# arkworks-rs/groth16

Measured on NVIDIA H100. Metric: groth16_proofs_per_sec_bls12_381_2^20, higher is better.
Workload: dtype u32 limbs (255-bit Fr / 381-bit Fq Montgomery integers)

## Files before the change

### groth16_b200/api.py

```python
from __future__ import annotations

import ctypes as C
from dataclasses import dataclass, field
from typing import List, Optional, Sequence, Tuple

import numpy as np

from . import _lib
from .codec import CurveCodec
from .params import CurveParams, get_curve


class SynthesisError(Exception):
    """ark_relations::r1cs::SynthesisError"""


class PolynomialDegreeTooLarge(SynthesisError):
    pass


class MalformedKey(SynthesisError):
    pass


# ... 278 lines not shown

    def prove_wait_raw(self, slot: int, out: np.ndarray):
        _check(self._lib.g16_prove_wait(self._ctx, slot, _ptr(out)))

    def prove_partial_submit_raw(self, slot: int, r_limbs: np.ndarray, z_ptr, flags: int):
        _check(self._lib.g16_prove_partial_submit(self._ctx, slot, _ptr(r_limbs), C.c_void_p(z_ptr), flags))

    def prove_partial_wait_raw(self, slot: int, out: np.ndarray):
        _check(self._lib.g16_prove_partial_wait(self._ctx, slot, _ptr(out)))

    def prove_partial_raw(self, r_limbs: np.ndarray, z_ptr, flags: int, out: np.ndarray):
        _check(self._lib.g16_prove_partial(self._ctx, _ptr(r_limbs), C.c_void_p(z_ptr), flags, _ptr(out)))

    def comm_unique_id(self) -> np.ndarray:
        out = np.zeros(256, dtype=np.uint8)
        _check(self._lib.g16_comm_unique_id(out.ctypes.data_as(C.c_void_p)))
        return out

    def comm_init(self, unique_id: np.ndarray, rank: int, world: int):
        uid = np.ascontiguousarray(unique_id, dtype=np.uint8)
        assert uid.size == 256
        _check(self._lib.g16_comm_init(self._ctx, uid.ctypes.data_as(C.c_void_p), rank, world))

    def prove_sharded_raw(self, r_limbs, s_limbs, z_ptr, flags: int, out: np.ndarray):
        _check(self._lib.g16_prove_sharded(self._ctx, _ptr(r_limbs), _ptr(s_limbs), C.c_void_p(z_ptr), flags, _ptr(out)))

    def prove_sharded_submit_raw(self, slot: int, r_limbs, s_limbs, z_ptr, flags: int):
        _check(self._lib.g16_prove_sharded_submit(self._ctx, slot, _ptr(r_limbs), _ptr(s_limbs), C.c_void_p(z_ptr), flags))

    def prove_sharded_wait_raw(self, slot: int, out: np.ndarray):
        _check(self._lib.g16_prove_sharded_wait(self._ctx, slot, _ptr(out)))

    def prove_assemble_prepare(self, r, s):
        self._asm_keep = (self._fr_arg(r), self._fr_arg(s))
        _check(self._lib.g16_prove_assemble_prepare(self._ctx, _ptr(self._asm_keep[0]), _ptr(self._asm_keep[1])))

    def prove_assemble(self, r, s, partials: np.ndarray) -> Proof:
        rr, ss = self._fr_arg(r), self._fr_arg(s)
        pl = self._lib.g16_partial_limbs(self._ctx)
        p = np.ascontiguousarray(partials, dtype=np.uint64).reshape(-1, pl)
        nq = self.nq
        out = np.zeros(8 * nq, dtype=np.uint64)
        _check(self._lib.g16_prove_assemble(self._ctx, _ptr(rr), _ptr(ss), _ptr(p), p.shape[0], _ptr(out)))
        return Proof(out[:2 * nq].copy(), out[2 * nq:6 * nq].copy(), out[6 * nq:].copy())

    def partial_limbs(self) -> int:
        return self._lib.g16_partial_limbs(self._ctx)

    def witness_map_from_matrices(self, matrices: Optional[ConstraintMatrices], num_inputs: int, num_constraints: int,
                                  full_assignment: np.ndarray) -> np.ndarray:
        if matrices is not None and matrices is not self._matrices:
            self.load_matrices(matrices)
        m = self._matrices
        z = np.ascontiguousarray(full_assignment, dtype=np.uint64).reshape(-1, 4)
        if z.shape[0] != m.num_instance_variables + m.num_witness_variables:
            raise ValueError("full_assignment has the wrong length")
        n = 1 << self._lib.g16_domain_log(self._ctx)
        h = np.zeros((n, 4), dtype=np.uint64)
        _check(self._lib.g16_witness_map(self._ctx, _ptr(z), 0, _ptr(h)))
        return h

    def timings(self) -> dict:
        t = _lib.Timings()
        _check(self._lib.g16_get_timings(self._ctx, C.byref(t)))
        names = ["h", "l", "a", "b_g1", "b_g2"]
        return dict(total_ms=t.total_ms, h2d_ms=t.h2d_ms, witness_map_ms=t.witness_map_ms,
                    msm_ms={n: t.msm_ms[i] for i, n in enumerate(names)},
                    msm_accum_ms={n: t.msm_accum_ms[i] for i, n in enumerate(names)},
                    msm_pairs={n: int(t.msm_pairs[i]) for i, n in enumerate(names)},
                    msm_entries={n: int(t.msm_entries[i]) for i, n in enumerate(names)},
                    msm_begin_ms={n: t.msm_begin_ms[i] for i, n in enumerate(names)},
                    msm_end_ms={n: t.msm_end_ms[i] for i, n in enumerate(names)},
                    host_finish_ms=t.host_finish_ms, launches=int(t.launches), h2d_bytes=int(t.h2d_bytes),
                    d2h_bytes=int(t.d2h_bytes))

    def set_option(self, key: str, value: int):
        _check(self._lib.g16_set_option(self._ctx, key.encode(), int(value)))

    def config(self) -> dict:
        c = _lib.Config()
        _check(self._lib.g16_get_config(self._ctx, C.byref(c)))
        d = {n: int(getattr(c, n)) for n, _ in _lib.Config._fields_ if n != "reserved"}
        R = d["ba_rounds_g1"]
        ba_mul = 6.0 + 3.0 / max(1, d["ba_m"])
        frac = 1.0 - 0.5 ** R
        d["imad_per_g1_entry_mul"] = frac * ba_mul + (1.0 - frac) * 10.0 if R > 0 else 10.0
        d["g1_accum_stage"] = (f"G1 bucket accumulation: {R} batched-affine rounds (ba_forward / ba_combine / ba_backward) + "
                               "msm_accum_l0<Fq> on the last list; one stage per G1 MSM" if R > 0 else
                               "msm_accum_l0<Fq> (G1 bucket accumulation, XYZZ mixed additions); one launch per G1 MSM")
        return d

    def _fr_arg(self, x) -> np.ndarray:
        if isinstance(x, (int, np.integer)):
            return np.ascontiguousarray(self.codec.fr.enc1(int(x)))
        return np.ascontiguousarray(x, dtype=np.uint64).reshape(4)
```

### groth16_b200/csrc/ec.cuh

```cuda
#pragma once
#include "fp.cuh"

#ifdef __CUDACC__
#define G16_HD_NOINLINE __host__ __device__ __noinline__
#else
#define G16_HD_NOINLINE
#endif

namespace g16 {

template <class P, int NR>
struct alignas(16) Fp2 {
  using B = Fp<P>;
  B c0, c1;
  G16_HD static Fp2 zero() { return {B::zero(), B::zero()}; }
  G16_HD static Fp2 one() { return {B::one(), B::zero()}; }
  G16_HD bool is_zero() const { return c0.is_zero() && c1.is_zero(); }
  G16_HD bool operator==(const Fp2& o) const { return c0 == o.c0 && c1 == o.c1; }
  G16_HD bool operator!=(const Fp2& o) const { return !(*this == o); }
  G16_HD static Fp2 add(const Fp2& a, const Fp2& b) { return {B::add(a.c0, b.c0), B::add(a.c1, b.c1)}; }
  G16_HD static Fp2 sub(const Fp2& a, const Fp2& b) { return {B::sub(a.c0, b.c0), B::sub(a.c1, b.c1)}; }
  G16_HD static Fp2 neg(const Fp2& a) { return {B::neg(a.c0), B::neg(a.c1)}; }
  G16_HD static Fp2 dbl(const Fp2& a) { return {B::dbl(a.c0), B::dbl(a.c1)}; }
  G16_HD static B mul_nr(const B& a) { return NR == 1 ? a : B::mul_small(a, NR); }
  G16_HD static Fp2 mul(const Fp2& a, const Fp2& b) {
    B v0 = B::mul(a.c0, b.c0);
    B v1 = B::mul(a.c1, b.c1);
    B s = B::mul(B::add(a.c0, a.c1), B::add(b.c0, b.c1));
    Fp2 r;
    r.c0 = B::sub(v0, mul_nr(v1));
    r.c1 = B::sub(B::sub(s, v0), v1);
    return r;
  }
  G16_HD static Fp2 sqr(const Fp2& a) {
    B t = B::mul(a.c0, a.c1);
    B s = B::mul(B::add(a.c0, a.c1), B::sub(a.c0, mul_nr(a.c1)));
    Fp2 r;
    r.c0 = (NR == 1) ? s : B::add(s, B::mul_small(t, NR - 1));
    r.c1 = B::dbl(t);
    return r;
  }
  G16_HD static Fp2 mul_small(const Fp2& a, int k) { return {B::mul_small(a.c0, k), B::mul_small(a.c1, k)}; }
  G16_HD static Fp2 inv(const Fp2& a) {
    B n = B::add(B::sqr(a.c0), mul_nr(B::sqr(a.c1)));
    B ni = B::inv(n);
    return {B::mul(a.c0, ni), B::neg(B::mul(a.c1, ni))};
  }
};

template <class F>
struct alignas(16) Affine {
  F x, y;
  G16_HD bool is_inf() const { return x.is_zero() && y.is_zero(); }
  G16_HD static Affine inf() { return {F::zero(), F::zero()}; }
};

template <class F>
struct alignas(16) XYZZ {
  F X, Y, ZZ, ZZZ;
  G16_HD bool is_inf() const { return ZZ.is_zero(); }
  G16_HD static XYZZ inf() { return {F::zero(), F::zero(), F::zero(), F::zero()}; }
  G16_HD static XYZZ from_affine(const Affine<F>& p) {
    if (p.is_inf()) return inf();
    return {p.x, p.y, F::one(), F::one()};
  }

  G16_HD_NOINLINE static XYZZ dbl_affine(const Affine<F>& p) {
    if (p.is_inf() || p.y.is_zero()) return inf();
    F U = F::dbl(p.y);
    F V = F::sqr(U);
    F W = F::mul(U, V);
    F S = F::mul(p.x, V);
    F XX = F::sqr(p.x);
    F M = F::add(F::dbl(XX), XX);
    XYZZ r;
    r.X = F::sub(F::sqr(M), F::dbl(S));
    r.Y = F::sub(F::mul(M, F::sub(S, r.X)), F::mul(W, p.y));
    r.ZZ = V;
    r.ZZZ = W;
    return r;
  }
  G16_HD_NOINLINE void dbl_inplace() {
    if (is_inf()) return;
    if (Y.is_zero()) { *this = inf(); return; }
    F U = F::dbl(Y);
    F V = F::sqr(U);
    F W = F::mul(U, V);
    F S = F::mul(X, V);
    F XX = F::sqr(X);
    F M = F::add(F::dbl(XX), XX);
    F X3 = F::sub(F::sqr(M), F::dbl(S));
    F Y3 = F::sub(F::mul(M, F::sub(S, X3)), F::mul(W, Y));
    X = X3;
    Y = Y3;
    ZZ = F::mul(V, ZZ);
    ZZZ = F::mul(W, ZZZ);
  }
  G16_HD_NOINLINE void madd(const Affine<F>& p_in, bool neg = false) { madd_inline(p_in, neg); }
  G16_HD void madd_inline(const Affine<F>& p_in, bool neg = false) {
    if (p_in.is_inf()) return;
    Affine<F> p = p_in;
    if (neg) p.y = F::neg(p.y);
    if (is_inf()) {
      X = p.x; Y = p.y; ZZ = F::one(); ZZZ = F::one();
      return;
    }
    F Pd = F::sub(F::mul(p.x, ZZ), X);
    F R = F::sub(F::mul(p.y, ZZZ), Y);
    if (Pd.is_zero()) {
      if (R.is_zero()) *this = dbl_affine(p);
      else *this = inf();
      return;
    }
    F PP = F::sqr(Pd);
    F PPP = F::mul(Pd, PP);
    F Q = F::mul(X, PP);
    F X3 = F::sub(F::sub(F::sqr(R), PPP), F::dbl(Q));
    Y = F::sub(F::mul(R, F::sub(Q, X3)), F::mul(Y, PPP));
    X = X3;
    ZZ = F::mul(ZZ, PP);
    ZZZ = F::mul(ZZZ, PPP);
  }
  template <class LX, class LY>
  G16_HD void madd_lazy(LX load_x, LY load_y, bool neg) {
    const F px = load_x();
    if (is_inf()) {
      F py = load_y();
      if (px.is_zero() && py.is_zero()) return;
      if (neg) py = F::neg(py);
      X = px; Y = py; ZZ = F::one(); ZZZ = F::one();
      return;
    }
    const F Pd = F::sub(F::mul(px, ZZ), X);
    F py = load_y();
    if (px.is_zero() && py.is_zero()) return;
    if (neg) py = F::neg(py);
    const F R = F::sub(F::mul(py, ZZZ), Y);
    if (Pd.is_zero()) {
      if (R.is_zero()) *this = dbl_affine(Affine<F>{px, py});
      else *this = inf();
      return;
    }
    const F PP = F::sqr(Pd);
    const F PPP = F::mul(Pd, PP);
    const F Q = F::mul(X, PP);
    const F X3 = F::sub(F::sub(F::sqr(R), PPP), F::dbl(Q));
    Y = F::sub(F::mul(R, F::sub(Q, X3)), F::mul(Y, PPP));
    X = X3;
    ZZ = F::mul(ZZ, PP);
    ZZZ = F::mul(ZZZ, PPP);
  }
  G16_HD_NOINLINE void add(const XYZZ& q) {
    if (q.is_inf()) return;
    if (is_inf()) { *this = q; return; }
    F U1 = F::mul(X, q.ZZ);
    F U2 = F::mul(q.X, ZZ);
    F S1 = F::mul(Y, q.ZZZ);
    F S2 = F::mul(q.Y, ZZZ);
    F Pd = F::sub(U2, U1);
    F R = F::sub(S2, S1);
    if (Pd.is_zero()) {
      if (R.is_zero()) dbl_inplace();
      else *this = inf();
      return;
    }
    F PP = F::sqr(Pd);
    F PPP = F::mul(Pd, PP);
    F Q = F::mul(U1, PP);
    F X3 = F::sub(F::sub(F::sqr(R), PPP), F::dbl(Q));
    Y = F::sub(F::mul(R, F::sub(Q, X3)), F::mul(S1, PPP));
    X = X3;
    ZZ = F::mul(F::mul(ZZ, q.ZZ), PP);
    ZZZ = F::mul(F::mul(ZZZ, q.ZZZ), PPP);
  }
  G16_HD void negate() { Y = F::neg(Y); }

  G16_HD_NOINLINE XYZZ mul_u32(const uint32_t* k, int nl) const {
    XYZZ r = inf();
    bool started = false;
    for (int i = nl * 32 - 1; i >= 0; i--) {
      if (started) r.dbl_inplace();
      if ((k[i >> 5] >> (i & 31)) & 1) {
        r.add(*this);
        started = true;
      }
    }
    return r;
  }
  G16_HD_NOINLINE Affine<F> to_affine() const {
    if (is_inf()) return Affine<F>::inf();
    F zi = F::inv(ZZZ);
    F z = F::mul(zi, ZZ);
    F zi2 = F::sqr(z);
    return {F::mul(X, zi2), F::mul(Y, zi)};
  }
};

}
```

### groth16_b200/csrc/fp.cuh

```cuda
#pragma once
#include <cstdint>
#include <cstring>
#include "g16_constants.h"

namespace g16 {

#if defined(__CUDA_ARCH__)
#define G16_PTX_PATH 1
namespace ptx {
__device__ __forceinline__ void add_cc(uint32_t& r, uint32_t a, uint32_t b) { asm volatile("add.cc.u32 %0, %1, %2;" : "=r"(r) : "r"(a), "r"(b)); }
__device__ __forceinline__ void addc_cc(uint32_t& r, uint32_t a, uint32_t b) { asm volatile("addc.cc.u32 %0, %1, %2;" : "=r"(r) : "r"(a), "r"(b)); }
__device__ __forceinline__ void addc(uint32_t& r, uint32_t a, uint32_t b) { asm volatile("addc.u32 %0, %1, %2;" : "=r"(r) : "r"(a), "r"(b)); }
__device__ __forceinline__ void sub_cc(uint32_t& r, uint32_t a, uint32_t b) { asm volatile("sub.cc.u32 %0, %1, %2;" : "=r"(r) : "r"(a), "r"(b)); }
__device__ __forceinline__ void subc_cc(uint32_t& r, uint32_t a, uint32_t b) { asm volatile("subc.cc.u32 %0, %1, %2;" : "=r"(r) : "r"(a), "r"(b)); }
__device__ __forceinline__ void subc(uint32_t& r, uint32_t a, uint32_t b) { asm volatile("subc.u32 %0, %1, %2;" : "=r"(r) : "r"(a), "r"(b)); }
__device__ __forceinline__ void mul_lo(uint32_t& r, uint32_t a, uint32_t b) { asm volatile("mul.lo.u32 %0, %1, %2;" : "=r"(r) : "r"(a), "r"(b)); }
__device__ __forceinline__ void mul_hi(uint32_t& r, uint32_t a, uint32_t b) { asm volatile("mul.hi.u32 %0, %1, %2;" : "=r"(r) : "r"(a), "r"(b)); }
__device__ __forceinline__ void mad_lo_cc(uint32_t& r, uint32_t a, uint32_t b, uint32_t c) { asm volatile("mad.lo.cc.u32 %0, %1, %2, %3;" : "=r"(r) : "r"(a), "r"(b), "r"(c)); }
__device__ __forceinline__ void madc_lo_cc(uint32_t& r, uint32_t a, uint32_t b, uint32_t c) { asm volatile("madc.lo.cc.u32 %0, %1, %2, %3;" : "=r"(r) : "r"(a), "r"(b), "r"(c)); }
__device__ __forceinline__ void madc_hi_cc(uint32_t& r, uint32_t a, uint32_t b, uint32_t c) { asm volatile("madc.hi.cc.u32 %0, %1, %2, %3;" : "=r"(r) : "r"(a), "r"(b), "r"(c)); }
__device__ __forceinline__ void madc_hi(uint32_t& r, uint32_t a, uint32_t b, uint32_t c) { asm volatile("madc.hi.u32 %0, %1, %2, %3;" : "=r"(r) : "r"(a), "r"(b), "r"(c)); }
}
#elif defined(G16_EMULATE_PTX)
#define G16_PTX_PATH 1
namespace ptx {
static thread_local uint32_t CF = 0;
inline void add_cc(uint32_t& r, uint32_t a, uint32_t b) { uint64_t t = (uint64_t)a + b; r = (uint32_t)t; CF = (uint32_t)(t >> 32); }
inline void addc_cc(uint32_t& r, uint32_t a, uint32_t b) { uint64_t t = (uint64_t)a + b + CF; r = (uint32_t)t; CF = (uint32_t)(t >> 32); }
inline void addc(uint32_t& r, uint32_t a, uint32_t b) { r = a + b + CF; }
inline void sub_cc(uint32_t& r, uint32_t a, uint32_t b) { uint64_t t = (uint64_t)a - b; r = (uint32_t)t; CF = (uint32_t)(t >> 63); }
inline void subc_cc(uint32_t& r, uint32_t a, uint32_t b) { uint64_t t = (uint64_t)a - b - CF; r = (uint32_t)t; CF = (uint32_t)(t >> 63); }
inline void subc(uint32_t& r, uint32_t a, uint32_t b) { r = a - b - CF; }
inline void mul_lo(uint32_t& r, uint32_t a, uint32_t b) { r = a * b; }
inline void mul_hi(uint32_t& r, uint32_t a, uint32_t b) { r = (uint32_t)(((uint64_t)a * b) >> 32); }
inline void mad_lo_cc(uint32_t& r, uint32_t a, uint32_t b, uint32_t c) { uint64_t t = (uint64_t)(uint32_t)(a * b) + c; r = (uint32_t)t; CF = (uint32_t)(t >> 32); }
inline void madc_lo_cc(uint32_t& r, uint32_t a, uint32_t b, uint32_t c) { uint64_t t = (uint64_t)(uint32_t)(a * b) + c + CF; r = (uint32_t)t; CF = (uint32_t)(t >> 32); }
inline void madc_hi_cc(uint32_t& r, uint32_t a, uint32_t b, uint32_t c) { uint64_t t = (((uint64_t)a * b) >> 32) + c + CF; r = (uint32_t)t; CF = (uint32_t)(t >> 32); }
inline void madc_hi(uint32_t& r, uint32_t a, uint32_t b, uint32_t c) { r = (uint32_t)(((uint64_t)a * b) >> 32) + c + CF; }
}
#endif

template <class P>
struct alignas(16) Fp {
  static constexpr int N = P::N;
  using Params = P;
  uint32_t v[N];

  G16_HD static Fp zero() {
    Fp r;
#pragma unroll
    for (int i = 0; i < N; i++) r.v[i] = 0;
    return r;
  }
  G16_HD static Fp one() {
    Fp r;
#pragma unroll
    for (int i = 0; i < N; i++) r.v[i] = P::one(i);
    return r;
  }
  G16_HD static Fp r2() {
    Fp r;
#pragma unroll
    for (int i = 0; i < N; i++) r.v[i] = P::r2(i);
    return r;
  }
  G16_HD static Fp modulus() {
    Fp r;
#pragma unroll
    for (int i = 0; i < N; i++) r.v[i] = P::mod(i);
    return r;
  }
  G16_HD bool is_zero() const {
    uint32_t acc = 0;
#pragma unroll
    for (int i = 0; i < N; i++) acc |= v[i];
    return acc == 0;
  }
  G16_HD bool operator==(const Fp& o) const {
    uint32_t acc = 0;
#pragma unroll
    for (int i = 0; i < N; i++) acc |= v[i] ^ o.v[i];
    return acc == 0;
  }
  G16_HD bool operator!=(const Fp& o) const { return !(*this == o); }

  G16_HD static Fp add(const Fp& a, const Fp& b) {
    Fp t, u;
#ifdef G16_PTX_PATH
    ptx::add_cc(t.v[0], a.v[0], b.v[0]);
#pragma unroll
    for (int i = 1; i < N - 1; i++) ptx::addc_cc(t.v[i], a.v[i], b.v[i]);
    ptx::addc(t.v[N - 1], a.v[N - 1], b.v[N - 1]);
    ptx::sub_cc(u.v[0], t.v[0], P::mod(0));
#pragma unroll
    for (int i = 1; i < N; i++) ptx::subc_cc(u.v[i], t.v[i], P::mod(i));
    uint32_t br;
    ptx::subc(br, 0, 0);
#pragma unroll
    for (int i = 0; i < N; i++) t.v[i] = br ? t.v[i] : u.v[i];
    return t;
#else
    uint64_t c = 0;
    for (int i = 0; i < N; i++) { c += (uint64_t)a.v[i] + b.v[i]; t.v[i] = (uint32_t)c; c >>= 32; }
    int64_t bw = 0;
    for (int i = 0; i < N; i++) { bw += (int64_t)t.v[i] - (int64_t)P::mod(i); u.v[i] = (uint32_t)bw; bw >>= 32; }
    return bw ? t : u;
#endif
  }
  G16_HD static Fp sub(const Fp& a, const Fp& b) {
    Fp t;
#ifdef G16_PTX_PATH
    ptx::sub_cc(t.v[0], a.v[0], b.v[0]);
#pragma unroll
    for (int i = 1; i < N; i++) ptx::subc_cc(t.v[i], a.v[i], b.v[i]);
    uint32_t br;
    ptx::subc(br, 0, 0);
    ptx::add_cc(t.v[0], t.v[0], P::mod(0) & br);
#pragma unroll
    for (int i = 1; i < N - 1; i++) ptx::addc_cc(t.v[i], t.v[i], P::mod(i) & br);
    ptx::addc(t.v[N - 1], t.v[N - 1], P::mod(N - 1) & br);
    return t;
#else
    int64_t bw = 0;
    for (int i = 0; i < N; i++) { bw += (int64_t)a.v[i] - (int64_t)b.v[i]; t.v[i] = (uint32_t)bw; bw >>= 32; }
    if (bw) {
      uint64_t c = 0;
      for (int i = 0; i < N; i++) { c += (uint64_t)t.v[i] + P::mod(i); t.v[i] = (uint32_t)c; c >>= 32; }
    }
    return t;
#endif
  }
  G16_HD static Fp neg(const Fp& a) { return a.is_zero() ? a : sub(modulus(), a); }
  G16_HD static Fp dbl(const Fp& a) { return add(a, a); }

#ifdef G16_PTX_PATH
  G16_HD static void cmad_row(uint32_t* acc, const uint32_t* x, uint32_t y) {
    ptx::mad_lo_cc(acc[0], x[0], y, acc[0]);
    ptx::madc_hi_cc(acc[1], x[0], y, acc[1]);
#pragma unroll
    for (int j = 2; j < N; j += 2) {
      ptx::madc_lo_cc(acc[j], x[j], y, acc[j]);
      ptx::madc_hi_cc(acc[j + 1], x[j], y, acc[j + 1]);
    }
  }
  template <int OFF>
  G16_HD static void cmad_row_mod(uint32_t* acc, uint32_t y) {
    ptx::mad_lo_cc(acc[0], P::mod(OFF), y, acc[0]);
    ptx::madc_hi_cc(acc[1], P::mod(OFF), y, acc[1]);
#pragma unroll
    for (int j = 2; j < N; j += 2) {
      ptx::madc_lo_cc(acc[j], P::mod(OFF + j), y, acc[j]);
      ptx::madc_hi_cc(acc[j + 1], P::mod(OFF + j), y, acc[j + 1]);
    }
  }
  template <bool FIRST>
  G16_HD static void mont_step(uint32_t* E, uint32_t* O, const uint32_t* a, uint32_t bi) {
    if (FIRST) {
#pragma unroll
      for (int j = 0; j < N; j += 2) {
        ptx::mul_lo(E[j], a[j], bi);
        ptx::mul_hi(E[j + 1], a[j], bi);
        ptx::mul_lo(O[j], a[j + 1], bi);
        ptx::mul_hi(O[j + 1], a[j + 1], bi);
      }
    } else {
      ptx::add_cc(E[0], E[0], O[1]);
#pragma unroll
      for (int j = 0; j < N - 2; j += 2) {
        ptx::madc_lo_cc(O[j], a[j + 1], bi, O[j + 2]);
        ptx::madc_hi_cc(O[j + 1], a[j + 1], bi, O[j + 3]);
      }
      ptx::madc_lo_cc(O[N - 2], a[N - 1], bi, 0);
      ptx::madc_hi(O[N - 1], a[N - 1], bi, 0);
      cmad_row(E, a, bi);
      ptx::addc(O[N - 1], O[N - 1], 0);
    }
    uint32_t m = E[0] * P::INV32;
    cmad_row_mod<1>(O, m);
    cmad_row_mod<0>(E, m);
    ptx::addc(O[N - 1], O[N - 1], 0);
  }
  G16_HD static Fp mul(const Fp& a, const Fp& b) {
    static_assert(N % 2 == 0, "even limb count required");
    uint32_t ev[N], od[N];
    mont_step<true>(ev, od, a.v, b.v[0]);
    mont_step<false>(od, ev, a.v, b.v[1]);
#pragma unroll
    for (int i = 2; i < N; i += 2) {
      mont_step<false>(ev, od, a.v, b.v[i]);
      mont_step<false>(od, ev, a.v, b.v[i + 1]);
    }
    Fp r;
    ptx::add_cc(r.v[0], od[1], ev[0]);
#pragma unroll
    for (int k = 1; k < N - 1; k++) ptx::addc_cc(r.v[k], od[k + 1], ev[k]);
    ptx::addc(r.v[N - 1], ev[N - 1], 0);
    return reduce_once(r);
  }
#else
  G16_HD static Fp mul(const Fp& a, const Fp& b) {
    constexpr int W = N / 2;
    uint64_t x[W], y[W], p[W], t[W + 2];
    memcpy(x, a.v, sizeof(x));
    memcpy(y, b.v, sizeof(y));
    for (int i = 0; i < W; i++) p[i] = (uint64_t)P::mod(2 * i) | ((uint64_t)P::mod(2 * i + 1) << 32);
    uint64_t inv = P::INV32;
    inv = inv * (2 + p[0] * inv);
    for (int i = 0; i < W + 2; i++) t[i] = 0;
    for (int i = 0; i < W; i++) {
      unsigned __int128 c = 0;
      for (int j = 0; j < W; j++) { c += (unsigned __int128)x[j] * y[i] + t[j]; t[j] = (uint64_t)c; c >>= 64; }
      c += t[W]; t[W] = (uint64_t)c; t[W + 1] = (uint64_t)(c >> 64);
      uint64_t m = t[0] * inv;
      c = (unsigned __int128)m * p[0] + t[0]; c >>= 64;
      for (int j = 1; j < W; j++) { c += (unsigned __int128)m * p[j] + t[j]; t[j - 1] = (uint64_t)c; c >>= 64; }
      c += t[W]; t[W - 1] = (uint64_t)c; t[W] = t[W + 1] + (uint64_t)(c >> 64);
    }
    Fp r;
    memcpy(r.v, t, sizeof(x));
    return reduce_once(r);
  }
#endif
  G16_HD static Fp sqr(const Fp& a) { return mul(a, a); }

  G16_HD static Fp reduce_once(const Fp& t) {
    Fp u;
#ifdef G16_PTX_PATH
    ptx::sub_cc(u.v[0], t.v[0], P::mod(0));
#pragma unroll
    for (int i = 1; i < N; i++) ptx::subc_cc(u.v[i], t.v[i], P::mod(i));
    uint32_t br;
    ptx::subc(br, 0, 0);
#pragma unroll
    for (int i = 0; i < N; i++) u.v[i] = br ? t.v[i] : u.v[i];
    return u;
#else
    int64_t bw = 0;
    for (int i = 0; i < N; i++) { bw += (int64_t)t.v[i] - (int64_t)P::mod(i); u.v[i] = (uint32_t)bw; bw >>= 32; }
    return bw ? t : u;
#endif
  }

  G16_HD static Fp from_mont(const Fp& a) {
    Fp o = zero();
    o.v[0] = 1;
    return mul(a, o);
  }
  G16_HD static Fp to_mont(const Fp& a) { return mul(a, r2()); }

  G16_HD static Fp mul_small(const Fp& a, int k) {
    Fp r = zero();
    Fp base = a;
    while (k) {
      if (k & 1) r = add(r, base);
      k >>= 1;
      if (k) base = dbl(base);
    }
    return r;
  }

  G16_HD static Fp pow(const Fp& a, const uint32_t* e, int nl) {
    Fp r = one();
    bool started = false;
    for (int i = nl * 32 - 1; i >= 0; i--) {
      if (started) r = sqr(r);
      if ((e[i >> 5] >> (i & 31)) & 1) {
        r = started ? mul(r, a) : a;
        started = true;
      }
    }
    return r;
  }
  G16_HD static Fp pow_u64(const Fp& a, uint64_t e) {
    uint32_t w[2] = {(uint32_t)e, (uint32_t)(e >> 32)};
    return pow(a, w, 2);
  }
  G16_HD static Fp inv(const Fp& a) {
    uint32_t e[N];
    uint64_t bw = 2;
    for (int i = 0; i < N; i++) {
      uint64_t m = P::mod(i);
      uint64_t d = m - bw;
      e[i] = (uint32_t)d;
      bw = (m < bw) ? 1 : 0;
    }
    return pow(a, e, N);
  }

  G16_HD friend Fp operator+(const Fp& a, const Fp& b) { return add(a, b); }
  G16_HD friend Fp operator-(const Fp& a, const Fp& b) { return sub(a, b); }
  G16_HD friend Fp operator*(const Fp& a, const Fp& b) { return mul(a, b); }
};

}
```

### groth16_b200/csrc/msm.cuh

```cuda
#pragma once
#include <cuda_runtime.h>
#include <algorithm>
#include <cstdlib>
#include "ec.cuh"

namespace g16 {

static constexpr uint32_t MSM_INVALID = 0xffffffffu;

struct MsmGeom {
  uint32_t n;
  int c;
  int W;
  int ne;
  int copies;
  uint32_t B;
  uint32_t nkeys;
  uint64_t max_entries;
  int k0;
  int ba;
  int ba_pad;
  int ba_m;
  int ba_G;
  int ba_gcd;
// ... 349 lines not shown
  const uint32_t tpo = jb.tpo;
  const uint32_t g = threadIdx.x / tpo, l = threadIdx.x % tpo;
  const uint32_t o = (blockIdx.x - jb.first_block) * (TPB / tpo) + g;
  XYZZ<F> acc = XYZZ<F>::inf();
  if (o < jb.n_out) {
    const uint32_t w = o / jb.per_win_out, r = o % jb.per_win_out;
    const XYZZ<F>* base = jb.in + (size_t)w * jb.win_stride + (size_t)r * jb.base_mul;
    for (uint32_t j = l; j < jb.len; j += tpo) acc.add(base[(size_t)j * jb.stride]);
  }
  for (uint32_t sft = tpo >> 1; sft > 0; sft >>= 1) {
    sm[threadIdx.x] = acc;
    __syncthreads();
    if (l < sft) acc.add(sm[threadIdx.x + sft]);
    __syncthreads();
  }
  if (l == 0 && o < jb.n_out) jb.out[o] = acc;
}

static constexpr int MSM_LEAF_LOG = 6;
struct MsmRedNode {
  int log_len, a0, a1;
  int child_r, child_c;
  size_t off;
  bool leaf;
};
struct MsmRedPlan {
  MsmRedNode nodes[16];
  int n_nodes = 0;
  size_t inner_pts = 0, leaf_pts = 0;
  int build(int log_len) {
    const int id = n_nodes++;
    MsmRedNode& nd = nodes[id];
    nd.log_len = log_len;
    nd.child_r = nd.child_c = -1;
    nd.leaf = log_len <= MSM_LEAF_LOG;
    nd.a0 = nd.a1 = 0;
    nd.off = 0;
    if (!nd.leaf) {
      const int a0 = log_len / 2, a1 = log_len - a0;
      nodes[id].a0 = a0;
      nodes[id].a1 = a1;
      const int r = build(a1);
      const int c = build(a0);
      nodes[id].child_r = r;
      nodes[id].child_c = c;
    }
    return id;
  }
  void layout() {
    inner_pts = leaf_pts = 0;
    for (int i = 1; i < n_nodes; i++)
      if (!nodes[i].leaf) { nodes[i].off = inner_pts; inner_pts += (size_t)1 << nodes[i].log_len; }
    for (int i = 0; i < n_nodes; i++)
      if (nodes[i].leaf) { nodes[i].off = leaf_pts; leaf_pts += (size_t)1 << nodes[i].log_len; }
  }
  void make(int m) { n_nodes = 0; build(m); layout(); }
};

template <class F>
__global__ void msm_inf_mask(const Affine<F>* __restrict__ bases, uint32_t n, uint8_t* __restrict__ mask) {
  const uint32_t i = blockIdx.x * blockDim.x + threadIdx.x;
  if (i >= n) return;
  const Affine<F> p = load_affine(bases, i);
  mask[i] = p.is_inf() ? 1 : 0;
}

static constexpr int MSM_MAX_COPIES = 20;
template <class F>
__global__ void __launch_bounds__(128) msm_precompute(const Affine<F>* in, uint32_t n, int copies, int shift,
                                                      Affine<F>* out) {
  const uint32_t i = blockIdx.x * blockDim.x + threadIdx.x;
  if (i >= n) return;
  const Affine<F> p = load_affine(in, i);
  out[i] = p;
  XYZZ<F> q = XYZZ<F>::from_affine(p);
  F Xs[MSM_MAX_COPIES], Ys[MSM_MAX_COPIES], ZZs[MSM_MAX_COPIES], ZZZs[MSM_MAX_COPIES], pref[MSM_MAX_COPIES];
  F acc = F::one();
  int live = 0;
  for (int j = 1; j < copies; j++) {
    for (int s = 0; s < shift; s++) q.dbl_inplace();
    if (q.is_inf()) break;
    Xs[j] = q.X; Ys[j] = q.Y; ZZs[j] = q.ZZ; ZZZs[j] = q.ZZZ;
    pref[j] = acc;
    acc = F::mul(acc, q.ZZZ);
    live = j;
  }
  for (int j = live + 1; j < copies; j++) out[(size_t)j * n + i] = Affine<F>::inf();
  if (live == 0) return;
  F inv = F::inv(acc);
  for (int j = live; j >= 1; j--) {
    const F zi = F::mul(inv, pref[j]);
    inv = F::mul(inv, ZZZs[j]);
    const F z = F::mul(zi, ZZs[j]);
    const F zi2 = F::sqr(z);
    Affine<F> a{F::mul(Xs[j], zi2), F::mul(Ys[j], zi)};
    out[(size_t)j * n + i] = a;
  }
}

struct DevBuf {
  void* p = nullptr;
  size_t cap = 0;
  cudaError_t reserve(size_t bytes) {
    if (bytes <= cap) return cudaSuccess;
    if (p) cudaFree(p);
    p = nullptr;
    cap = 0;
    cudaError_t e = cudaMalloc(&p, bytes);
    if (e == cudaSuccess) cap = bytes;
    return e;
  }
  void release() {
    if (p) cudaFree(p);
    p = nullptr;
    cap = 0;
  }
  template <class T>
  T* as() const { return reinterpret_cast<T*>(p); }
};

static constexpr int MSM_KF = 4;
static constexpr int MSM_TAIL_S = 2048;

static constexpr int MSM_BA_MAX_ROUNDS = 6;
struct MsmBaPlan {
  int R = 0, pad = 0;
  uint64_t len[MSM_BA_MAX_ROUNDS + 1] = {0};
  uint32_t m[MSM_BA_MAX_ROUNDS] = {0};
  uint64_t threads_max = 0;
  int k0_final = 0;
  void make(const MsmGeom& g) {
    R = g.ba < 0 ? 0 : (g.ba > MSM_BA_MAX_ROUNDS ? MSM_BA_MAX_ROUNDS : g.ba);
    pad = g.ba_pad > R ? (g.ba_pad > MSM_BA_MAX_ROUNDS ? MSM_BA_MAX_ROUNDS : g.ba_pad) : R;
    len[0] = pad > 0 ? ((g.max_entries + (uint64_t)g.nkeys * ((1u << pad) - 1)) >> pad) << pad : g.max_entries;
    threads_max = 0;
    for (int r = 0; r < R; r++) {
      len[r + 1] = len[r] >> 1;
      uint32_t mm = (uint32_t)(g.ba_m < 1 ? 1 : g.ba_m);
      while (mm > 4 && len[r + 1] / mm < 200000) mm >>= 1;
      m[r] = mm;
      const uint64_t T = ba_threads(len[r + 1], mm);
      if (T > threads_max) threads_max = T;
    }
    k0_final = g.k0 >> R;
    if (k0_final < 8) k0_final = g.k0 < 8 ? g.k0 : 8;
  }
  uint64_t l0_threads(const MsmGeom& g) const {
    return R > 0 ? (len[R] + k0_final - 1) / k0_final : (g.max_entries + g.k0 - 1) / g.k0;
  }
  template <class F>
  uint64_t extra_bytes() const {
    if (R == 0) return 0;
    return len[1] * (sizeof(F) + sizeof(Affine<F>)) + (R > 1 ? len[2] * sizeof(Affine<F>) : 0) + 2 * threads_max * sizeof(F);
  }
};

template <class F>
struct MsmWorkspace {
  DevBuf counters, offsets, blocktot, sidx, skey, buckets, pk0, pp0, pk1, pp1, pending, red_inner, red_leaf;
  DevBuf ba_pre, ba_prod, ba_pre2, ba_l0, ba_l1;
  MsmBaPlan bap;
  MsmRedPlan plan;
  int plan_m = -1, plan_ne = 0;
  XYZZ<F>* h_leaf = nullptr;
  size_t h_cap = 0;
  uint32_t* h_total = nullptr;
  cudaError_t prepare(const MsmGeom& g) {
    cudaError_t e;
    bap.make(g);
    const uint64_t T0 = bap.l0_threads(g);
    const uint64_t S1 = 2 * T0;
    const uint64_t T1 = msm_level_threads(S1, MSM_KF);
    const uint64_t S2 = 2 * T1;
#define G16_TRY(x) if ((e = (x)) != cudaSuccess) return e
    if (bap.R > 0) {
      G16_TRY(ba_pre.reserve(bap.len[1] * sizeof(F) + 16));
      G16_TRY(ba_prod.reserve(bap.threads_max * sizeof(F) + 16));
      G16_TRY(ba_pre2.reserve(bap.threads_max * sizeof(F) + 16));
// ... 326 lines not shown
```

Baseline: 23.51.

## Add dedicated wide squaring and lazy-reduction Fq2 multiplication

Fp squaring now uses a dedicated PTX sqr_wide that computes the cross products once and doubles them, followed by a separate Montgomery redc, in place of a general multiply of a value by itself. Fq2 multiplication now keeps the Karatsuba partial products at double width and reduces only twice, adding NR*p^2 so the subtraction cannot go negative. In exchange it adds wide-integer helpers and a mul_reduced alias, which the curve formulas now call for base-field multiplies. The aim is fewer IMAD instructions in G1/G2 point arithmetic for MSM, at the cost of larger register footprints.

```diff
diff --git a/groth16_b200/api.py b/groth16_b200/api.py
--- a/groth16_b200/api.py
+++ b/groth16_b200/api.py
@@ -384,9 +384,12 @@
         _check(self._lib.g16_get_config(self._ctx, C.byref(c)))
         d = {n: int(getattr(c, n)) for n, _ in _lib.Config._fields_ if n != "reserved"}
         R = d["ba_rounds_g1"]
-        ba_mul = 6.0 + 3.0 / max(1, d["ba_m"])
+        nl = 2 * self.nq
+        sqr = (nl * (nl + 1) / 2 + nl * nl) / (2 * nl * nl)
+        ba_mul = 5.0 + sqr + 3.0 / max(1, d["ba_m"])
+        madd = 8.0 + 2.0 * sqr
         frac = 1.0 - 0.5 ** R
-        d["imad_per_g1_entry_mul"] = frac * ba_mul + (1.0 - frac) * 10.0 if R > 0 else 10.0
+        d["imad_per_g1_entry_mul"] = frac * ba_mul + (1.0 - frac) * madd if R > 0 else madd
         d["g1_accum_stage"] = (f"G1 bucket accumulation: {R} batched-affine rounds (ba_forward / ba_combine / ba_backward) + "
                                "msm_accum_l0<Fq> on the last list; one stage per G1 MSM" if R > 0 else
                                "msm_accum_l0<Fq> (G1 bucket accumulation, XYZZ mixed additions); one launch per G1 MSM")
diff --git a/groth16_b200/csrc/ec.cuh b/groth16_b200/csrc/ec.cuh
--- a/groth16_b200/csrc/ec.cuh
+++ b/groth16_b200/csrc/ec.cuh
@@ -23,7 +23,55 @@
   G16_HD static Fp2 neg(const Fp2& a) { return {B::neg(a.c0), B::neg(a.c1)}; }
   G16_HD static Fp2 dbl(const Fp2& a) { return {B::dbl(a.c0), B::dbl(a.c1)}; }
   G16_HD static B mul_nr(const B& a) { return NR == 1 ? a : B::mul_small(a, NR); }
+
+  using Wide = typename B::Wide;
+  G16_HD static constexpr Wide nr_p2_limbs() {
+    Wide r{};
+    for (int i = 0; i < B::N; i++) {
+      uint64_t c = 0;
+      for (int j = 0; j < B::N; j++) {
+        c += (uint64_t)P::mod(i) * P::mod(j) + r.v[i + j];
+        r.v[i + j] = (uint32_t)c;
+        c >>= 32;
+      }
+      r.v[i + B::N] = (uint32_t)c;
+    }
+    uint64_t c = 0;
+    for (int k = 0; k < 2 * B::N; k++) {
+      c += (uint64_t)r.v[k] * NR;
+      r.v[k] = (uint32_t)c;
+      c >>= 32;
+    }
+    return r;
+  }
+  G16_HD static constexpr uint32_t nr_p2(int k) {
+    constexpr Wide t = nr_p2_limbs();
+    return t.v[k];
+  }
   G16_HD static Fp2 mul(const Fp2& a, const Fp2& b) {
+    static_assert(32 * B::N - P::BITS >= (NR + 1 <= 2 ? 1 : NR + 1 <= 4 ? 2 : NR + 1 <= 8 ? 3 : 4),
+                  "lazy Fq2 reduction needs (NR + 1) p < 2^(32N)");
+    Wide t = B::mul_wide(B::add_nored(a.c0, a.c1), B::add_nored(b.c0, b.c1));
+    Wide w;
+    {
+      const Wide v0 = B::mul_wide(a.c0, b.c0);
+      t = B::wide_sub(t, v0);
+      Wide k;
+#pragma unroll
+      for (int i = 0; i < 2 * B::N; i++) k.v[i] = nr_p2(i);
+      w = B::wide_add(v0, k);
+    }
+    {
+      const Wide v1 = B::mul_wide(a.c1, b.c1);
+      t = B::wide_sub(t, v1);
+      w = sub_nr_times(w, v1);
+    }
+    Fp2 r;
+    r.c0 = B::redc(w);
+    r.c1 = B::redc(t);
+    return r;
+  }
+  G16_HD static Fp2 mul_reduced(const Fp2& a, const Fp2& b) {
     B v0 = B::mul(a.c0, b.c0);
     B v1 = B::mul(a.c1, b.c1);
     B s = B::mul(B::add(a.c0, a.c1), B::add(b.c0, b.c1));
@@ -31,6 +79,17 @@
     r.c0 = B::sub(v0, mul_nr(v1));
     r.c1 = B::sub(B::sub(s, v0), v1);
     return r;
+  }
+  G16_HD static Wide sub_nr_times(Wide w, const Wide& x) {
+#pragma unroll
+    for (int s = 0; s < 8; s++) {
+      if (!((NR >> s) & 1)) continue;
+      Wide y;
+#pragma unroll
+      for (int k = 2 * B::N - 1; k >= 0; k--) y.v[k] = s == 0 ? x.v[k] : (x.v[k] << s) | (k ? x.v[k - 1] >> (32 - s) : 0u);
+      w = B::wide_sub(w, y);
+    }
+    return w;
   }
   G16_HD static Fp2 sqr(const Fp2& a) {
     B t = B::mul(a.c0, a.c1);
@@ -69,13 +128,13 @@
     if (p.is_inf() || p.y.is_zero()) return inf();
     F U = F::dbl(p.y);
     F V = F::sqr(U);
-    F W = F::mul(U, V);
-    F S = F::mul(p.x, V);
+    F W = F::mul_reduced(U, V);
+    F S = F::mul_reduced(p.x, V);
     F XX = F::sqr(p.x);
     F M = F::add(F::dbl(XX), XX);
     XYZZ r;
     r.X = F::sub(F::sqr(M), F::dbl(S));
-    r.Y = F::sub(F::mul(M, F::sub(S, r.X)), F::mul(W, p.y));
+    r.Y = F::sub(F::mul_reduced(M, F::sub(S, r.X)), F::mul_reduced(W, p.y));
     r.ZZ = V;
     r.ZZZ = W;
     return r;
@@ -85,16 +144,16 @@
     if (Y.is_zero()) { *this = inf(); return; }
     F U = F::dbl(Y);
     F V = F::sqr(U);
-    F W = F::mul(U, V);
-    F S = F::mul(X, V);
+    F W = F::mul_reduced(U, V);
+    F S = F::mul_reduced(X, V);
     F XX = F::sqr(X);
     F M = F::add(F::dbl(XX), XX);
     F X3 = F::sub(F::sqr(M), F::dbl(S));
-    F Y3 = F::sub(F::mul(M, F::sub(S, X3)), F::mul(W, Y));
+    F Y3 = F::sub(F::mul_reduced(M, F::sub(S, X3)), F::mul_reduced(W, Y));
     X = X3;
     Y = Y3;
-    ZZ = F::mul(V, ZZ);
-    ZZZ = F::mul(W, ZZZ);
+    ZZ = F::mul_reduced(V, ZZ);
+    ZZZ = F::mul_reduced(W, ZZZ);
   }
   G16_HD_NOINLINE void madd(const Affine<F>& p_in, bool neg = false) { madd_inline(p_in, neg); }
   G16_HD void madd_inline(const Affine<F>& p_in, bool neg = false) {
@@ -105,21 +164,21 @@
       X = p.x; Y = p.y; ZZ = F::one(); ZZZ = F::one();
       return;
     }
-    F Pd = F::sub(F::mul(p.x, ZZ), X);
-    F R = F::sub(F::mul(p.y, ZZZ), Y);
+    F Pd = F::sub(F::mul_reduced(p.x, ZZ), X);
+    F R = F::sub(F::mul_reduced(p.y, ZZZ), Y);
     if (Pd.is_zero()) {
       if (R.is_zero()) *this = dbl_affine(p);
       else *this = inf();
       return;
     }
     F PP = F::sqr(Pd);
-    F PPP = F::mul(Pd, PP);
-    F Q = F::mul(X, PP);
+    F PPP = F::mul_reduced(Pd, PP);
+    F Q = F::mul_reduced(X, PP);
     F X3 = F::sub(F::sub(F::sqr(R), PPP), F::dbl(Q));
-    Y = F::sub(F::mul(R, F::sub(Q, X3)), F::mul(Y, PPP));
-    X = X3;
-    ZZ = F::mul(ZZ, PP);
-    ZZZ = F::mul(ZZZ, PPP);
+    Y = F::sub(F::mul_reduced(R, F::sub(Q, X3)), F::mul_reduced(Y, PPP));
+    X = X3;
+    ZZ = F::mul_reduced(ZZ, PP);
+    ZZZ = F::mul_reduced(ZZZ, PPP);
   }
   template <class LX, class LY>
   G16_HD void madd_lazy(LX load_x, LY load_y, bool neg) {
@@ -131,32 +190,32 @@
       X = px; Y = py; ZZ = F::one(); ZZZ = F::one();
       return;
     }
-    const F Pd = F::sub(F::mul(px, ZZ), X);
+    const F Pd = F::sub(F::mul_reduced(px, ZZ), X);
     F py = load_y();
     if (px.is_zero() && py.is_zero()) return;
     if (neg) py = F::neg(py);
-    const F R = F::sub(F::mul(py, ZZZ), Y);
+    const F R = F::sub(F::mul_reduced(py, ZZZ), Y);
     if (Pd.is_zero()) {
       if (R.is_zero()) *this = dbl_affine(Affine<F>{px, py});
       else *this = inf();
       return;
     }
     const F PP = F::sqr(Pd);
-    const F PPP = F::mul(Pd, PP);
-    const F Q = F::mul(X, PP);
+    const F PPP = F::mul_reduced(Pd, PP);
+    const F Q = F::mul_reduced(X, PP);
     const F X3 = F::sub(F::sub(F::sqr(R), PPP), F::dbl(Q));
-    Y = F::sub(F::mul(R, F::sub(Q, X3)), F::mul(Y, PPP));
-    X = X3;
-    ZZ = F::mul(ZZ, PP);
-    ZZZ = F::mul(ZZZ, PPP);
+    Y = F::sub(F::mul_reduced(R, F::sub(Q, X3)), F::mul_reduced(Y, PPP));
+    X = X3;
+    ZZ = F::mul_reduced(ZZ, PP);
+    ZZZ = F::mul_reduced(ZZZ, PPP);
   }
   G16_HD_NOINLINE void add(const XYZZ& q) {
     if (q.is_inf()) return;
     if (is_inf()) { *this = q; return; }
-    F U1 = F::mul(X, q.ZZ);
-    F U2 = F::mul(q.X, ZZ);
-    F S1 = F::mul(Y, q.ZZZ);
-    F S2 = F::mul(q.Y, ZZZ);
+    F U1 = F::mul_reduced(X, q.ZZ);
+    F U2 = F::mul_reduced(q.X, ZZ);
+    F S1 = F::mul_reduced(Y, q.ZZZ);
+    F S2 = F::mul_reduced(q.Y, ZZZ);
     F Pd = F::sub(U2, U1);
     F R = F::sub(S2, S1);
     if (Pd.is_zero()) {
@@ -165,13 +224,13 @@
       return;
     }
     F PP = F::sqr(Pd);
-    F PPP = F::mul(Pd, PP);
-    F Q = F::mul(U1, PP);
+    F PPP = F::mul_reduced(Pd, PP);
+    F Q = F::mul_reduced(U1, PP);
     F X3 = F::sub(F::sub(F::sqr(R), PPP), F::dbl(Q));
-    Y = F::sub(F::mul(R, F::sub(Q, X3)), F::mul(S1, PPP));
-    X = X3;
-    ZZ = F::mul(F::mul(ZZ, q.ZZ), PP);
-    ZZZ = F::mul(F::mul(ZZZ, q.ZZZ), PPP);
+    Y = F::sub(F::mul_reduced(R, F::sub(Q, X3)), F::mul_reduced(S1, PPP));
+    X = X3;
+    ZZ = F::mul_reduced(F::mul_reduced(ZZ, q.ZZ), PP);
+    ZZZ = F::mul_reduced(F::mul_reduced(ZZZ, q.ZZZ), PPP);
   }
   G16_HD void negate() { Y = F::neg(Y); }
 
@@ -190,9 +249,9 @@
   G16_HD_NOINLINE Affine<F> to_affine() const {
     if (is_inf()) return Affine<F>::inf();
     F zi = F::inv(ZZZ);
-    F z = F::mul(zi, ZZ);
+    F z = F::mul_reduced(zi, ZZ);
     F zi2 = F::sqr(z);
-    return {F::mul(X, zi2), F::mul(Y, zi)};
+    return {F::mul_reduced(X, zi2), F::mul_reduced(Y, zi)};
   }
 };
 
diff --git a/groth16_b200/csrc/fp.cuh b/groth16_b200/csrc/fp.cuh
--- a/groth16_b200/csrc/fp.cuh
+++ b/groth16_b200/csrc/fp.cuh
@@ -45,6 +45,7 @@
   static constexpr int N = P::N;
   using Params = P;
   uint32_t v[N];
+  struct Wide { uint32_t v[2 * N]; };
 
   G16_HD static Fp zero() {
     Fp r;
@@ -197,7 +198,222 @@
     ptx::addc(r.v[N - 1], ev[N - 1], 0);
     return reduce_once(r);
   }
+
+  G16_HD static void wide_step(uint32_t* E, uint32_t* O, const uint32_t* a, uint32_t bi) {
+    ptx::add_cc(E[0], E[0], O[1]);
+#pragma unroll
+    for (int j = 0; j < N - 2; j += 2) {
+      ptx::madc_lo_cc(O[j], a[j + 1], bi, O[j + 2]);
+      ptx::madc_hi_cc(O[j + 1], a[j + 1], bi, O[j + 3]);
+    }
+    ptx::madc_lo_cc(O[N - 2], a[N - 1], bi, 0);
+    ptx::madc_hi(O[N - 1], a[N - 1], bi, 0);
+    cmad_row(E, a, bi);
+    ptx::addc(O[N - 1], O[N - 1], 0);
+  }
+  G16_HD static Wide mul_wide(const Fp& a, const Fp& b) {
+    uint32_t ev[N], od[N];
+    Wide r;
+#pragma unroll
+    for (int j = 0; j < N; j += 2) {
+      ptx::mul_lo(ev[j], a.v[j], b.v[0]);
+      ptx::mul_hi(ev[j + 1], a.v[j], b.v[0]);
+      ptx::mul_lo(od[j], a.v[j + 1], b.v[0]);
+      ptx::mul_hi(od[j + 1], a.v[j + 1], b.v[0]);
+    }
+    r.v[0] = ev[0];
+#pragma unroll
+    for (int i = 1; i < N; i += 2) {
+      wide_step(od, ev, a.v, b.v[i]);
+      r.v[i] = od[0];
+      if (i + 1 < N) {
+        wide_step(ev, od, a.v, b.v[i + 1]);
+        r.v[i + 1] = ev[0];
+      }
+    }
+    ptx::add_cc(r.v[N], od[1], ev[0]);
+#pragma unroll
+    for (int k = 1; k < N - 1; k++) ptx::addc_cc(r.v[N + k], od[k + 1], ev[k]);
+    ptx::addc(r.v[2 * N - 1], ev[N - 1], 0);
+    return r;
+  }
+  G16_HD static Wide sqr_wide(const Fp& a) {
+    uint32_t ev[2 * N], od[2 * N];
+#pragma unroll
+    for (int k = 1; k < N; k += 2) {
+      ptx::mul_lo(od[k], a.v[0], a.v[k]);
+      ptx::mul_hi(od[k + 1], a.v[0], a.v[k]);
+    }
+#pragma unroll
+    for (int k = 2; k < N; k += 2) {
+      ptx::mul_lo(ev[k], a.v[0], a.v[k]);
+      ptx::mul_hi(ev[k + 1], a.v[0], a.v[k]);
+    }
+#pragma unroll
+    for (int i = 1; i < N - 1; i++) {
+      uint32_t* top = (i & 1) ? ev : od;
+      uint32_t* low = (i & 1) ? od : ev;
+      const int k_top = (i & 1) ? i + 2 : i + 1;
+      const int k_low = (i & 1) ? i + 1 : i + 2;
+      if (k_top == N - 1) {
+        ptx::mul_lo(top[i + k_top], a.v[i], a.v[k_top]);
+        ptx::mul_hi(top[i + k_top + 1], a.v[i], a.v[k_top]);
+      } else {
+        ptx::mad_lo_cc(top[i + k_top], a.v[i], a.v[k_top], top[i + k_top]);
+        ptx::madc_hi_cc(top[i + k_top + 1], a.v[i], a.v[k_top], top[i + k_top + 1]);
+#pragma unroll
+        for (int k = k_top + 2; k < N - 1; k += 2) {
+          ptx::madc_lo_cc(top[i + k], a.v[i], a.v[k], top[i + k]);
+          ptx::madc_hi_cc(top[i + k + 1], a.v[i], a.v[k], top[i + k + 1]);
+        }
+        ptx::madc_lo_cc(top[i + N - 1], a.v[i], a.v[N - 1], 0);
+        ptx::madc_hi(top[i + N], a.v[i], a.v[N - 1], 0);
+      }
+      if (k_low < N - 1) {
+        ptx::mad_lo_cc(low[i + k_low], a.v[i], a.v[k_low], low[i + k_low]);
+        ptx::madc_hi_cc(low[i + k_low + 1], a.v[i], a.v[k_low], low[i + k_low + 1]);
+#pragma unroll
+        for (int k = k_low + 2; k < N - 1; k += 2) {
+          ptx::madc_lo_cc(low[i + k], a.v[i], a.v[k], low[i + k]);
+          ptx::madc_hi_cc(low[i + k + 1], a.v[i], a.v[k], low[i + k + 1]);
+        }
+        ptx::addc(top[i + N], top[i + N], 0);
+      }
+    }
+    uint32_t s[2 * N];
+    s[0] = 0;
+    s[1] = od[1];
+    ptx::add_cc(s[2], od[2], ev[2]);
+#pragma unroll
+    for (int k = 3; k < 2 * N - 2; k++) ptx::addc_cc(s[k], od[k], ev[k]);
+    ptx::addc_cc(s[2 * N - 2], od[2 * N - 2], 0);
+    ptx::addc(s[2 * N - 1], 0, 0);
+#pragma unroll
+    for (int k = 2 * N - 1; k > 0; k--) s[k] = (s[k] << 1) | (s[k - 1] >> 31);
+    Wide r;
+    ptx::mad_lo_cc(r.v[0], a.v[0], a.v[0], s[0]);
+    ptx::madc_hi_cc(r.v[1], a.v[0], a.v[0], s[1]);
+#pragma unroll
+    for (int j = 1; j < N - 1; j++) {
+      ptx::madc_lo_cc(r.v[2 * j], a.v[j], a.v[j], s[2 * j]);
+      ptx::madc_hi_cc(r.v[2 * j + 1], a.v[j], a.v[j], s[2 * j + 1]);
+    }
+    ptx::madc_lo_cc(r.v[2 * N - 2], a.v[N - 1], a.v[N - 1], s[2 * N - 2]);
+    ptx::madc_hi(r.v[2 * N - 1], a.v[N - 1], a.v[N - 1], s[2 * N - 1]);
+    return r;
+  }
+  G16_HD static void redc_step(uint32_t* E, uint32_t* O) {
+    ptx::add_cc(E[0], E[0], O[1]);
+    uint32_t m;
+    ptx::mul_lo(m, E[0], P::INV32);
+    ptx::madc_lo_cc(O[0], P::mod(1), m, O[2]);
+    ptx::madc_hi_cc(O[1], P::mod(1), m, O[3]);
+#pragma unroll
+    for (int j = 2; j < N - 2; j += 2) {
+      ptx::madc_lo_cc(O[j], P::mod(j + 1), m, O[j + 2]);
+      ptx::madc_hi_cc(O[j + 1], P::mod(j + 1), m, O[j + 3]);
+    }
+    ptx::madc_lo_cc(O[N - 2], P::mod(N - 1), m, 0);
+    ptx::madc_hi(O[N - 1], P::mod(N - 1), m, 0);
+    cmad_row_mod<0>(E, m);
+    ptx::addc(O[N - 1], O[N - 1], 0);
+  }
+  G16_HD static Fp redc(const Wide& t) {
+    uint32_t ev[N], od[N];
+#pragma unroll
+    for (int j = 0; j < N; j++) ev[j] = t.v[j];
+    const uint32_t m = ev[0] * P::INV32;
+#pragma unroll
+    for (int j = 0; j < N; j += 2) {
+      ptx::mul_lo(od[j], P::mod(j + 1), m);
+      ptx::mul_hi(od[j + 1], P::mod(j + 1), m);
+    }
+    cmad_row_mod<0>(ev, m);
+    ptx::addc(od[N - 1], od[N - 1], 0);
+    redc_step(od, ev);
+#pragma unroll
+    for (int i = 2; i < N; i += 2) {
+      redc_step(ev, od);
+      redc_step(od, ev);
+    }
+    Fp r;
+    ptx::add_cc(r.v[0], od[1], ev[0]);
+#pragma unroll
+    for (int k = 1; k < N - 1; k++) ptx::addc_cc(r.v[k], od[k + 1], ev[k]);
+    ptx::addc(r.v[N - 1], ev[N - 1], 0);
+    ptx::add_cc(r.v[0], r.v[0], t.v[N]);
+#pragma unroll
+    for (int k = 1; k < N - 1; k++) ptx::addc_cc(r.v[k], r.v[k], t.v[N + k]);
+    ptx::addc(r.v[N - 1], r.v[N - 1], t.v[2 * N - 1]);
+    return reduce_once(r);
+  }
+  G16_HD static Wide wide_add(const Wide& a, const Wide& b) {
+    Wide r;
+    ptx::add_cc(r.v[0], a.v[0], b.v[0]);
+#pragma unroll
+    for (int k = 1; k < 2 * N - 1; k++) ptx::addc_cc(r.v[k], a.v[k], b.v[k]);
+    ptx::addc(r.v[2 * N - 1], a.v[2 * N - 1], b.v[2 * N - 1]);
+    return r;
+  }
+  G16_HD static Wide wide_sub(const Wide& a, const Wide& b) {
+    Wide r;
+    ptx::sub_cc(r.v[0], a.v[0], b.v[0]);
+#pragma unroll
+    for (int k = 1; k < 2 * N - 1; k++) ptx::subc_cc(r.v[k], a.v[k], b.v[k]);
+    ptx::subc(r.v[2 * N - 1], a.v[2 * N - 1], b.v[2 * N - 1]);
+    return r;
+  }
+  G16_HD static Fp add_nored(const Fp& a, const Fp& b) {
+    Fp r;
+    ptx::add_cc(r.v[0], a.v[0], b.v[0]);
+#pragma unroll
+    for (int i = 1; i < N - 1; i++) ptx::addc_cc(r.v[i], a.v[i], b.v[i]);
+    ptx::addc(r.v[N - 1], a.v[N - 1], b.v[N - 1]);
+    return r;
+  }
 #else
+  G16_HD static Wide mul_wide(const Fp& a, const Fp& b) {
+    Wide r;
+    for (int k = 0; k < 2 * N; k++) r.v[k] = 0;
+    for (int i = 0; i < N; i++) {
+      uint64_t c = 0;
+      for (int j = 0; j < N; j++) { c += (uint64_t)a.v[j] * b.v[i] + r.v[i + j]; r.v[i + j] = (uint32_t)c; c >>= 32; }
+      r.v[i + N] = (uint32_t)c;
+    }
+    return r;
+  }
+  G16_HD static Wide sqr_wide(const Fp& a) { return mul_wide(a, a); }
+  G16_HD static Fp redc(const Wide& t) {
+    uint32_t w[2 * N];
+    for (int k = 0; k < 2 * N; k++) w[k] = t.v[k];
+    for (int i = 0; i < N; i++) {
+      const uint32_t m = w[i] * P::INV32;
+      uint64_t c = 0;
+      for (int j = 0; j < N; j++) { c += (uint64_t)m * P::mod(j) + w[i + j]; w[i + j] = (uint32_t)c; c >>= 32; }
+      for (int k = i + N; c && k < 2 * N; k++) { c += w[k]; w[k] = (uint32_t)c; c >>= 32; }
+    }
+    Fp r;
+    for (int j = 0; j < N; j++) r.v[j] = w[N + j];
+    return reduce_once(r);
+  }
+  G16_HD static Wide wide_add(const Wide& a, const Wide& b) {
+    Wide r;
+    uint64_t c = 0;
+    for (int k = 0; k < 2 * N; k++) { c += (uint64_t)a.v[k] + b.v[k]; r.v[k] = (uint32_t)c; c >>= 32; }
+    return r;
+  }
+  G16_HD static Wide wide_sub(const Wide& a, const Wide& b) {
+    Wide r;
+    int64_t bw = 0;
+    for (int k = 0; k < 2 * N; k++) { bw += (int64_t)a.v[k] - (int64_t)b.v[k]; r.v[k] = (uint32_t)bw; bw >>= 32; }
+    return r;
+  }
+  G16_HD static Fp add_nored(const Fp& a, const Fp& b) {
+    Fp r;
+    uint64_t c = 0;
+    for (int i = 0; i < N; i++) { c += (uint64_t)a.v[i] + b.v[i]; r.v[i] = (uint32_t)c; c >>= 32; }
+    return r;
+  }
   G16_HD static Fp mul(const Fp& a, const Fp& b) {
     constexpr int W = N / 2;
     uint64_t x[W], y[W], p[W], t[W + 2];
@@ -221,7 +437,11 @@
     return reduce_once(r);
   }
 #endif
+#ifdef G16_PTX_PATH
+  G16_HD static Fp sqr(const Fp& a) { return redc(sqr_wide(a)); }
+#else
   G16_HD static Fp sqr(const Fp& a) { return mul(a, a); }
+#endif
 
   G16_HD static Fp reduce_once(const Fp& t) {
     Fp u;
@@ -287,6 +507,8 @@
     return pow(a, e, N);
   }
 
+  G16_HD static Fp mul_reduced(const Fp& a, const Fp& b) { return mul(a, b); }
+
   G16_HD friend Fp operator+(const Fp& a, const Fp& b) { return add(a, b); }
   G16_HD friend Fp operator-(const Fp& a, const Fp& b) { return sub(a, b); }
   G16_HD friend Fp operator*(const Fp& a, const Fp& b) { return mul(a, b); }
diff --git a/groth16_b200/csrc/msm.cuh b/groth16_b200/csrc/msm.cuh
--- a/groth16_b200/csrc/msm.cuh
+++ b/groth16_b200/csrc/msm.cuh
@@ -455,18 +455,18 @@
     if (q.is_inf()) break;
     Xs[j] = q.X; Ys[j] = q.Y; ZZs[j] = q.ZZ; ZZZs[j] = q.ZZZ;
     pref[j] = acc;
-    acc = F::mul(acc, q.ZZZ);
+    acc = F::mul_reduced(acc, q.ZZZ);
     live = j;
   }
   for (int j = live + 1; j < copies; j++) out[(size_t)j * n + i] = Affine<F>::inf();
   if (live == 0) return;
   F inv = F::inv(acc);
   for (int j = live; j >= 1; j--) {
-    const F zi = F::mul(inv, pref[j]);
-    inv = F::mul(inv, ZZZs[j]);
-    const F z = F::mul(zi, ZZs[j]);
+    const F zi = F::mul_reduced(inv, pref[j]);
+    inv = F::mul_reduced(inv, ZZZs[j]);
+    const F z = F::mul_reduced(zi, ZZs[j]);
     const F zi2 = F::sqr(z);
-    Affine<F> a{F::mul(Xs[j], zi2), F::mul(Ys[j], zi)};
+    Affine<F> a{F::mul_reduced(Xs[j], zi2), F::mul_reduced(Ys[j], zi)};
     out[(size_t)j * n + i] = a;
   }
 }
```

New measurement: 24.14 (median of 6 runs). +2.7%, better.
